# iagostorch/VVC-Affine-GPU

Measured on AMD Instinct MI355X. Metric: candidate CU-blocks/s at 1080p QP32; bit-exact CPMV/cost match vs reference, higher is better.
Workload: dtype int32; 1 GPU; 1920x1080 QP32, 2 frames, 2-CPMV affine only (FULL+HALF CUs); resolution=1920x1080, qp=32, sequence_frames=2, sequence_pairs=3, pocs_rank0=2, modes=2cp, parallelism=frame-shard x1 (a sequence of its own per rank)

## Files before the change

vvc-affine-gpu_amd/csrc/vame_engine.hip:

```cpp
#include <hip/hip_ext.h>
#include <hip/hip_runtime.h>

#include <algorithm>
#include <cstdio>
#include <cstdlib>
#include <cstring>
#include <vector>

#include "../../include/vame.h"
#include "vame_kernel.h"
#include "vame_bipred.h"
#include "vame_birefine.h"

#if VAME_SPLIT_TU
namespace vame {
VAME_2CP_KERNELS(extern)
}
#endif

using namespace vame;

static_assert(sizeof(vame_cpmvs) == 28, "Cpmvs layout (typedef.h)");
static_assert(sizeof(vame_cpmvs_dev) == 28, "Cpmvs layout (typedef.h)");
static_assert(sizeof(vame_mc_cu) == sizeof(McCu) && VAME_MC_MAX_CUS == kMcMaxCus, "vame_mc_cu layout");
static_assert(sizeof(vame_mc_bicu) == sizeof(McBiCu) && sizeof(McBiCu) == 80, "vame_mc_bicu layout");

static thread_local char g_hip_err[256] = "";

#define VAME_HIP(x)                                                               \
  do {                                                                            \
    hipError_t e_ = (x);                                                          \
    if (e_ != hipSuccess) {                                                       \
      snprintf(g_hip_err, sizeof(g_hip_err), "%s (%s:%d)", hipGetErrorString(e_), \
               __FILE__, __LINE__);                                               \
      return VAME_E_DEVICE;                                                       \
    }                                                                             \
  } while (0)

constexpr int kTimingClasses = 7;

struct vame_ctx {
  int device, W, H, nCtus, ctusPerRow;
  Item* dQuad = nullptr;
  int quadOff[4][3] = {}, quadN[4][3] = {};
  Item* dBig1 = nullptr;
  Item* dHalf = nullptr;
  Item* dHalfW = nullptr;
  Item* dHalfH = nullptr;
  int nBig1 = 0, nHalf = 0, nHalfW = 0, nHalfH = 0;
  int32_t* bestS = nullptr;
  size_t bestOff[4] = {0, 0, 0, 0};
  int maxPairs = kMaxPairs;
  hipEvent_t bestEv = nullptr;
  hipStream_t bestStream = nullptr;
  bool bestPending = false;
  int32_t* dOrder[2] = {nullptr, nullptr};
  int groupCombos[2] = {408, 408}, nChunks[2] = {1, 1}, cpp[2] = {0, 0};
  int streams = 2;
  hipStream_t side = nullptr;
  hipStream_t side2 = nullptr;
  hipEvent_t evFork = nullptr, evJoin = nullptr, evJoin2 = nullptr;
  int valueSync = 1;
  uint32_t* syncWord = nullptr;
  uint32_t joinSeq = 0;
  int timing = 0;
  bool prof = false;
  std::vector<std::pair<hipEvent_t, hipEvent_t>> ev[kTimingClasses];
  size_t evUsed[kTimingClasses] = {};
  std::vector<struct PackSeg> packSegs;
  struct PackSeg* dPackSegs = nullptr;
  size_t dPackCap = 0;
  hipEvent_t packEv = nullptr;
  int32_t* mcScratch = nullptr;
  int32_t* partScratch = nullptr;
  BiCand* biCands = nullptr;
  int32_t* biGroupCand = nullptr;
  int64_t* biPairSatd = nullptr;
// ... 76 lines not shown
    it.nCu = (int16_t)(t * stride + n);
  }
  return it;
}
Item make_coop_item(int rx, int ry, const std::vector<CuDesc>& cus, int threads) {
  return make_coop_item(rx, ry, std::vector<std::vector<CuDesc>>{cus}, threads);
}

Item make_auto_item(int rx, int ry, const std::vector<std::vector<CuDesc>>& tasks, int sbl) {
  Item it;
  memset(&it, 0, sizeof(it));
  it.rx = (int16_t)rx;
  it.ry = (int16_t)ry;
  it.coop = sbl == 2 ? 2 | 4 : 2;
  if (tasks.empty() || (int)tasks.size() > kMaxTasks) abort();
  it.nTasks = (int16_t)tasks.size();
  it.nCu = (int16_t)(tasks.size() * kTaskCu);
  for (size_t t = 0; t < tasks.size(); t++) {
    const int lanes = nsb_of(tasks[t][0]) / sbl;
    const int n = (int)tasks[t].size();
    for (auto& c : tasks[t])
      if (nsb_of(c) / sbl != lanes) abort();
    if (n * lanes > 64 || lanes < 16 || n > kTaskCu) abort();
    for (int i = 0; i < n; i++) set_slot(it.cu[t * kTaskCu + i], tasks[t][i]);
    it.cu[t * kTaskCu].taskCus = (uint8_t)n;
    it.cu[t * kTaskCu].taskLogL = (uint16_t)ilog2(lanes);
  }
  return it;
}

#ifndef VAME_Q2_TASKS
#define VAME_Q2_TASKS 16
#endif
size_t pack_autonomous(int qx, int qy, std::vector<CuDesc> cus, std::vector<Item>& out, int sbl) {
  const int perItem = sbl == 2 ? VAME_Q2_TASKS : kMaxTasks;
  std::stable_sort(cus.begin(), cus.end(),
                   [](const CuDesc& a, const CuDesc& b) { return nsb_of(a) > nsb_of(b); });
  std::vector<std::vector<CuDesc>> waves;
  for (auto& c : cus) {
    if (waves.empty() || nsb_of(waves.back()[0]) != nsb_of(c) || (int)waves.back().size() == kTaskCu ||
        (int)(waves.back().size() + 1) * nsb_of(c) / sbl > 64)
      waves.push_back({});
    waves.back().push_back(c);
  }
  for (size_t w = 0; w < waves.size(); w += perItem) {
    std::vector<std::vector<CuDesc>> grp(waves.begin() + w,
                                         waves.begin() + std::min(waves.size(), w + perItem));
    out.push_back(make_auto_item(qx, qy, grp, sbl));
  }
  return (waves.size() + perItem - 1) / perItem;
}

struct QuadSet {
  std::vector<Item> full, half, both;
};

void build_templates(std::vector<Item>& big, std::vector<Item>& halfItems, QuadSet& q1, QuadSet* q2) {
  for (int g = 0; g < kFullGroups; g++) {
    const int w = kFullW[g], h = kFullH[g], n = (kCtu * kCtu) / (w * h), cols = kCtu / w;
    if (w == 128 || h == 128) {
      std::vector<CuDesc> c;
      for (int k = 0; k < n; k++) c.push_back({(k % cols) * w, (k / cols) * h, w, h, 0, kFullStride[g] + k});
      if (w != h) {
        if (VAME_ABLATE & 256) continue;
        for (auto& cu : c) {
          Item it = make_coop_item(cu.x, cu.y, {cu}, Cfg<kKindHalf>::THREADS);
          it.rw = (int16_t)w;
          it.rh = (int16_t)h;
          halfItems.push_back(it);
        }
      } else {
        big.push_back(make_coop_item(0, 0, c, Cfg<kKindCtu>::THREADS));
      }
    }
  }
  const int max1 = q2 ? 16 : 64, min2 = 32, max2 = 128;
  struct Both {
    std::vector<Item> coop, autos;
    std::vector<int> rank;
  } both1, both2;
  for (int q = 0; q < 4; q++) {
    const int qx = (q & 1) * 64, qy = (q >> 1) * 64;
    auto inq = [&](int x, int y) { return x >= qx && x < qx + 64 && y >= qy && y < qy + 64; };
    std::vector<CuDesc> a1[2], a2[2];
    std::vector<std::vector<CuDesc>> coop[2];
    auto place = [&](const std::vector<CuDesc>& c, int align) {
      if (c.empty()) return;
      const int nsb = nsb_of(c[0]);
      if (nsb <= max1)
        a1[align].insert(a1[align].end(), c.begin(), c.end());
      else if (q2 && nsb >= min2 && nsb <= max2)
        a2[align].insert(a2[align].end(), c.begin(), c.end());
      else
        coop[align].push_back(c);
    };
    for (int g = 0; g < kFullGroups; g++) {
      const int w = kFullW[g], h = kFullH[g], n = (kCtu * kCtu) / (w * h), cols = kCtu / w;
      if (w == 128 || h == 128) continue;
      std::vector<CuDesc> c;
      for (int k = 0; k < n; k++) {
        const int x = (k % cols) * w, y = (k / cols) * h;
        if (inq(x, y)) c.push_back({x, y, w, h, 0, kFullStride[g] + k});
      }
      place(c, 0);
    }
    std::vector<CuDesc> halfBig;
    for (int g = 0; g < kHalfGroups; g++) {
      std::vector<CuDesc> c;
      for (int k = 0; k < kHalfN[g]; k++) {
        const int x = kHalfX8[g][k] * 8, y = kHalfY8[g][k] * 8;
        if (!inq(x, y)) continue;
        if (x + kHalfW[g] > qx + 64 || y + kHalfH[g] > qy + 64) abort();
        c.push_back({x, y, kHalfW[g], kHalfH[g], 1, kHalfStride[g] + k});
      }
      if (!c.empty() && nsb_of(c[0]) > max1 && !(q2 && nsb_of(c[0]) <= max2))
        halfBig.insert(halfBig.end(), c.begin(), c.end());
      else
        place(c, 1);
    }
    if (!halfBig.empty()) coop[1].push_back(halfBig);
    for (int al = 0; al < 2; al++) {
      std::vector<Item>& o1 = al ? q1.half : q1.full;
      if (!coop[al].empty()) o1.push_back(make_coop_item(qx, qy, coop[al], Cfg<kKindQuad>::THREADS));
      pack_autonomous(qx, qy, a1[al], o1, 1);
      if (q2) pack_autonomous(qx, qy, a2[al], al ? q2->half : q2->full, 2);
    }
    std::vector<std::vector<CuDesc>> t(coop[0]);
    t.insert(t.end(), coop[1].begin(), coop[1].end());
    if (!t.empty()) both1.coop.push_back(make_coop_item(qx, qy, t, Cfg<kKindQuad>::THREADS));
    for (int k = 0; k < (q2 ? 2 : 1); k++) {
      Both& b = k ? both2 : both1;
      std::vector<CuDesc> cus(k ? a2[0] : a1[0]);
      const std::vector<CuDesc>& h = k ? a2[1] : a1[1];
      cus.insert(cus.end(), h.begin(), h.end());
      const size_t n = pack_autonomous(qx, qy, cus, b.autos, k ? 2 : 1);
      for (size_t i = 0; i < n; i++) b.rank.push_back((int)i);
    }
  }
  for (int k = 0; k < (q2 ? 2 : 1); k++) {
    Both& b = k ? both2 : both1;
    std::vector<Item>& out = k ? q2->both : q1.both;
    out = b.coop;
    std::vector<size_t> idx(b.autos.size());
    for (size_t i = 0; i < idx.size(); i++) idx[i] = i;
    std::stable_sort(idx.begin(), idx.end(), [&](size_t x, size_t y) { return b.rank[x] < b.rank[y]; });
    for (size_t i : idx) out.push_back(b.autos[i]);
  }
}

size_t best_layout(const vame_ctx* c, int pairs, size_t off[4]) {
  const size_t per = (size_t)pairs * c->nCtus * 5;
  int nq2 = 0;
  for (int a = 0; a < 3; a++) nq2 = std::max({nq2, c->quadN[1][a], c->quadN[3][a]});
  off[0] = 0;
  off[1] = off[0] + per * c->nBig1 * Cfg<kKindCtu2>::NSB;
  off[2] = off[1] + per * c->nHalfW * Cfg<kKindHalf2W>::NSB;
  off[3] = off[2] + per * c->nHalfH * Cfg<kKindHalf2H>::NSB;
  return off[3] + per * nq2 * Cfg<kKindQuad2>::NSB;
}

int alloc_best(vame_ctx* c, int pairs) {
  if (c->bestS) {
    VAME_HIP(hipDeviceSynchronize());
    VAME_HIP(hipFree(c->bestS));
    c->bestS = nullptr;
  }
  c->bestPending = false;
  const size_t words = best_layout(c, pairs, c->bestOff);
  if (hipMalloc(&c->bestS, words * sizeof(int32_t)) != hipSuccess) {
    (void)hipGetLastError();
    c->bestS = nullptr;
    return VAME_E_NOMEM;
  }
  c->maxPairs = pairs;
  return VAME_OK;
}

void fill_common(KParams& kp, const vame_ctx* c, int extra) {
  kp.W = c->W;
  kp.H = c->H;
  kp.nCtus = c->nCtus;
// ... 180 lines not shown
      return VAME_OK;
    }
    if (half_merged(mode)) {
      KParams kh = kp;
      kh.items = c->dHalfW;
      kh.nItems = c->nHalfW + c->nHalfH;
      kh.bestS = c->bestS + c->bestOff[1];
      const unsigned grid = block_grid(c, 1, kh);
      hipEvent_t t0, t1;
      VAME_TRY(events(4, t0, t1));
      VAME_HIP(launch_kernel(kernel_for<kKindHalf2W + 100>(mode), grid, Cfg<kKindHalf2W>::THREADS, stream, t0,
                             t1, order_flag(), kh, capture));
      return VAME_OK;
    }
    for (int o = 0; o < 2; o++) {
      KParams kh = kp;
      kh.items = o ? c->dHalfH : c->dHalfW;
      kh.nItems = o ? c->nHalfH : c->nHalfW;
      kh.bestS = c->bestS + c->bestOff[1 + o];
      const unsigned grid = block_grid(c, 1, kh);
      hipEvent_t t0, t1;
      VAME_TRY(events(4 + o, t0, t1));
      VAME_HIP(launch_kernel(o ? kernel_for<kKindHalf2H>(mode) : kernel_for<kKindHalf2W>(mode), grid,
                             Cfg<kKindHalf2W>::THREADS, stream, t0, t1, order_flag(), kh, capture));
    }
    return VAME_OK;
  };
  const int aset = quadFull && quadHalf ? 2 : quadFull ? 0 : 1;
  auto quad = [&](const KParams& kp, int set, hipStream_t s) -> int {
    KParams kq = kp;
    kq.items = c->dQuad + c->quadOff[set][aset];
    kq.nItems = c->quadN[set][aset];
    kq.bestS = c->bestS + c->bestOff[3];
    const unsigned grid = block_grid(c, 0, kq);
    hipEvent_t t0, t1;
    VAME_TRY(events(set == 1 ? 6 : 0, t0, t1));
    if (set == 1)
      VAME_HIP(launch_kernel(kernel_for<kKindQuad2>(mode), grid, Cfg<kKindQuad2>::THREADS, s, t0, t1, order_flag(),
                             kq, capture));
    else
      VAME_HIP(launch_kernel(quad_kernel(c->prof, mode), grid, Cfg<kKindQuad>::THREADS, s, t0, t1, order_flag(),
                             kq, capture));
    return VAME_OK;
  };
  const bool anyQuad = quadFull || quadHalf;
  const bool kSplit = VAME_SPLIT == 1 || (VAME_SPLIT == 3 && mode != 1);
  auto quads = [&](const KParams& kp, hipStream_t s1) -> int {
    if (c->prof || VAME_SPLIT == 0) return quad(kp, 2, sQuad);
    if (!kSplit) return quad(kp, 3, sQuad);
    VAME_TRY(quad(kp, 1, sQuad));
    if (s1 == sQuad || !fork) VAME_TRY(quad(kp, 0, s1));
    return VAME_OK;
  };
  auto all = [&]() -> int {
    for (const KParams& kp : kps) {
      if (!fork && anyQuad) VAME_TRY(quads(kp, stream));
      if (bigItems) {
        VAME_TRY(big(kp));
        VAME_TRY(half(kp));
      }
      if (fork) {
        VAME_TRY(quads(kp, kQ1Side ? sQuad : stream));
        if (!kQ1Side && !c->prof && kSplit) VAME_TRY(quad(kp, 0, c->side2 ? c->side2 : stream));
      }
    }
    return fork ? join() : VAME_OK;
  };
// ... 42 lines not shown
    *ncu = (kCtu * kCtu) / (*w * *h);
    *stride = kFullStride[g];
    for (int k = 0; k < *ncu; k++) {
      xs[k] = (k % (kCtu / *w)) * *w;
      ys[k] = (k / (kCtu / *w)) * *h;
    }
    return VAME_OK;
  }
  if (align == 1 && g >= 0 && g < kHalfGroups) {
    *w = kHalfW[g];
    *h = kHalfH[g];
    *ncu = kHalfN[g];
    *stride = kHalfStride[g];
    for (int k = 0; k < *ncu; k++) {
      xs[k] = kHalfX8[g][k] * 8;
      ys[k] = kHalfY8[g][k] * 8;
    }
    return VAME_OK;
  }
  return VAME_E_INVALID;
}

int vame_create(vame_ctx** out, int device, int width, int height) {
  if (!out) return VAME_E_INVALID;
  *out = nullptr;
  const int nCtus = num_ctus(width, height);
  if (!nCtus) return VAME_E_INVALID;
  int ndev = 0;
  VAME_HIP(hipGetDeviceCount(&ndev));
  if (device < 0 || device >= ndev) return VAME_E_INVALID;
  DeviceGuard guard(device);
  VAME_HIP(guard.err);
  std::vector<Item> big1, hf, bigP, hfP;
  QuadSet qs[4];
  build_templates(big1, hf, qs[0], &qs[1]);
  build_templates(bigP, hfP, qs[2], nullptr);
  for (int a = 0; a < 3; a++) {
    const std::vector<Item>& v1 = a == 0 ? qs[0].full : a == 1 ? qs[0].half : qs[0].both;
    const std::vector<Item>& v2 = a == 0 ? qs[1].full : a == 1 ? qs[1].half : qs[1].both;
    std::vector<Item>& m = a == 0 ? qs[3].full : a == 1 ? qs[3].half : qs[3].both;
    for (const Item& it : v1)
      if (it.coop & 1) m.push_back(it);
    m.insert(m.end(), v2.begin(), v2.end());
    for (const Item& it : v1)
      if (!(it.coop & 1)) m.push_back(it);
  }
  std::vector<Item> hfw, hfh;
  for (const Item& it : hf) (it.cu[0].lw > it.cu[0].lh ? hfw : hfh).push_back(it);
  if (big1.size() != 1 || (!(VAME_ABLATE & 256) && (hfw.size() != 2 || hfh.size() != 2))) return VAME_E_INVALID;
  vame_ctx* c = new vame_ctx();
  c->device = device;
  c->W = width;
  c->H = height;
  c->nCtus = nCtus;
  c->ctusPerRow = (width + kCtu - 1) / kCtu;
  c->nBig1 = (int)big1.size();
  c->nHalf = (int)hf.size();
  c->nHalfW = (int)hfw.size();
  c->nHalfH = (int)hfh.size();
  std::vector<Item> quad;
  for (int k = 0; k < 4; k++)
    for (int a = 0; a < 3; a++) {
      const std::vector<Item>& v = a == 0 ? qs[k].full : a == 1 ? qs[k].half : qs[k].both;
      c->quadOff[k][a] = (int)quad.size();
      c->quadN[k][a] = (int)v.size();
      quad.insert(quad.end(), v.begin(), v.end());
    }
  c->streams = env_int("VAME_STREAMS", 2) == 1 ? 1 : 2;
  c->valueSync = env_int("VAME_SYNC", 1) != 0 ? 1 : 0;
  c->groupCombos[0] = c->groupCombos[1] = std::max(8, env_int("VAME_GROUP_COMBOS", 408));
  hipError_t e = hipSuccess;
  auto upload = [&](Item*& d, const std::vector<Item>& v) {
    if (e == hipSuccess && !v.empty()) e = hipMalloc(&d, v.size() * sizeof(Item));
    if (e == hipSuccess && !v.empty()) e = hipMemcpy(d, v.data(), v.size() * sizeof(Item), hipMemcpyHostToDevice);
  };
  upload(c->dQuad, quad);
  upload(c->dBig1, big1);
  upload(c->dHalf, hf);
  {
    std::vector<Item> hwh(hfw);
    hwh.insert(hwh.end(), hfh.begin(), hfh.end());
    upload(c->dHalfW, hwh);
    if (c->dHalfW) c->dHalfH = c->dHalfW + hfw.size();
  }
  for (int k = 0; k < 2 && e == hipSuccess; k++) {
    const std::vector<int32_t> order = build_order(nCtus, c->ctusPerRow, c->groupCombos[k], c->nChunks[k], c->cpp[k]);
    e = hipMalloc(&c->dOrder[k], order.size() * sizeof(int32_t));
    if (e == hipSuccess)
      e = hipMemcpy(c->dOrder[k], order.data(), order.size() * sizeof(int32_t), hipMemcpyHostToDevice);
  }
  if (e == hipSuccess && c->streams == 2) e = hipStreamCreateWithFlags(&c->side, hipStreamNonBlocking);
  if (e == hipSuccess && c->streams == 2 && VAME_SPLIT != 2 && VAME_Q1_SIDE == 2)
    e = hipStreamCreateWithFlags(&c->side2, hipStreamNonBlocking);
  if (e == hipSuccess) e = hipEventCreateWithFlags(&c->evJoin, hipEventDisableTiming);
  if (e == hipSuccess) e = hipEventCreateWithFlags(&c->evJoin2, hipEventDisableTiming);
  if (e == hipSuccess) e = hipEventCreateWithFlags(&c->evFork, hipEventDisableTiming);
  if (e == hipSuccess) e = hipEventCreateWithFlags(&c->bestEv, hipEventDisableTiming);
  if (e == hipSuccess && c->valueSync) {
    if (hipExtMallocWithFlags(reinterpret_cast<void**>(&c->syncWord), 8, hipMallocSignalMemory) != hipSuccess ||
        hipMemset(c->syncWord, 0, 8) != hipSuccess) {
      (void)hipGetLastError();
      if (c->syncWord) (void)hipFree(c->syncWord);
      c->syncWord = nullptr;
      c->valueSync = 0;
// ... 330 lines not shown
  if (reinterpret_cast<uintptr_t>(cur) & 7) return VAME_E_INVALID;
  BiRefineParams p;
  memset(&p, 0, sizeof(p));
  for (int r = 0; r < nrefs; r++) {
    if (!refs[r] || (reinterpret_cast<uintptr_t>(refs[r]) & 3)) return VAME_E_INVALID;
    p.refs[r] = refs[r];
  }
  if (c->prof) return VAME_E_UNSUPPORTED;
  if (max_cus == 0) return VAME_OK;
  DeviceGuard guard(c->device);
  VAME_HIP(guard.err);
  p.cur = cur;
  p.cus = reinterpret_cast<const McBiCu*>(cus);
  p.out = reinterpret_cast<McBiCu*>(out);
  p.cost = cost;
  p.bad = bad;
  p.maxCus = max_cus;
  p.nrefs = nrefs;
  p.W = c->W;
  p.H = c->H;
  p.rounds = rounds;
  p.lambda = lambda;
  p.ncusDev = ncus_dev;
  VAME_HIP(birefine_launch(p, (hipStream_t)stream));
  return VAME_OK;
}

int vame_template_coverage(int half128, int align, int32_t* hits, int32_t* items3) {
  if (!hits || (align != 0 && align != 1) || half128 == 0) return VAME_E_INVALID;
  std::vector<Item> big, hf, bigP, hfP;
  QuadSet q1, q2, qp;
  build_templates(big, hf, q1, &q2);
  build_templates(bigP, hfP, qp, nullptr);
  std::vector<Item> qf(q1.full), qh(q1.half), qb(q1.both);
  qf.insert(qf.end(), q2.full.begin(), q2.full.end());
  qh.insert(qh.end(), q2.half.begin(), q2.half.end());
  qb.insert(qb.end(), q2.both.begin(), q2.both.end());
  for (const std::vector<Item>* pv : {&qp.full, &qp.half, &qp.both}) {
    std::vector<int32_t> a((size_t)(align ? kHalfCusPerCtu : kFullCusPerCtu), 0),
        b((size_t)(align ? kHalfCusPerCtu : kFullCusPerCtu), 0);
    const std::vector<Item>& split = pv == &qp.full ? qf : pv == &qp.half ? qh : qb;
    for (int k = 0; k < 2; k++)
      for (const Item& it : k ? split : *pv)
        for (int i = 0; i < it.nCu; i++)
          if (it.cu[i].lw != 0 && it.cu[i].align == align) (k ? b : a)[it.cu[i].outOff]++;
    if (a != b) return VAME_E_INVALID;
  }
  const int n = align ? kHalfCusPerCtu : kFullCusPerCtu;
  std::vector<int32_t> both(n, 0);
  for (int i = 0; i < n; i++) hits[i] = 0;
  for (const auto* v : {&big, &hf, &qf, &qh, &qb})
    for (const Item& it : *v)
      for (int k = 0; k < it.nCu; k++) {
        const CuSlot& s = it.cu[k];
        if (s.lw == 0 || s.align != align) continue;
        if (s.outOff >= n) return VAME_E_INVALID;
        (v == &qb ? both[s.outOff] : hits[s.outOff])++;
      }
  for (const auto* v : {&big, &hf})
    for (const Item& it : *v)
      for (int k = 0; k < it.nCu; k++)
        if (it.cu[k].lw != 0 && it.cu[k].align == align) both[it.cu[k].outOff]++;
  for (int i = 0; i < n; i++)
    if (both[i] != hits[i]) return VAME_E_INVALID;
  if (items3) {
    items3[0] = (int32_t)qb.size();
// ... 157 lines not shown
    case VAME_E_DEVICE: return "HIP runtime error";
    case VAME_E_NOMEM: return "out of memory";
    case VAME_E_UNSUPPORTED: return "unsupported";
    default: return "unknown error";
  }
}

const char* vame_last_hip_error(void) { return g_hip_err; }

#if VAME_PHASE_TIMING
int vame_debug_phase_cycles(unsigned long long* out, int reset) {
  if (!out) return VAME_E_INVALID;
  VAME_HIP(hipDeviceSynchronize());
  VAME_HIP(hipMemcpyFromSymbol(out, HIP_SYMBOL(g_phase_cycles), sizeof(g_phase_cycles)));
  if (reset) {
    unsigned long long z[7 * kPhSlots] = {};
    VAME_HIP(hipMemcpyToSymbol(HIP_SYMBOL(g_phase_cycles), z, sizeof(z)));
  }
  return VAME_OK;
}
#endif
#if VAME_COUNT_PRED
int vame_debug_pred_count(unsigned long long* out20, int reset) {
  if (!out20) return VAME_E_INVALID;
  VAME_HIP(hipDeviceSynchronize());
  VAME_HIP(hipMemcpyFromSymbol(out20, HIP_SYMBOL(g_pred_count), sizeof(unsigned long long) * 20));
  if (reset) {
    unsigned long long z[20] = {};
    VAME_HIP(hipMemcpyToSymbol(HIP_SYMBOL(g_pred_count), z, sizeof(z)));
  }
  return VAME_OK;
}
#endif
const char* vame_version(void) { return "vame 0.1 (gfx950)"; }

}
```

vvc-affine-gpu_amd/csrc/vame_kernel.h:

```cpp
#pragma once
#include <hip/hip_runtime.h>

#include "vame_tables.h"

namespace vame {

constexpr int kMaxCu = 16;
constexpr int kMaxTasks = 16;
constexpr int kTaskCu = 4;
constexpr int kItemCu = kMaxTasks * kTaskCu;
constexpr int kThreads = 256;
constexpr int kNumMom = 24;
constexpr int kNumVal2 = 14;

struct vame_cpmvs_dev {
  int32_t ncps, ltx, lty, rtx, rty, lbx, lby;
};

struct CuSlot {
  uint8_t x, y;
  uint8_t lw : 4, lh : 4;
  uint8_t align : 1;
  uint8_t taskCus : 5;
  uint16_t outOff : 9;
// ... 86 lines not shown
#define PH_MARK(i) { const unsigned long long t_ = __builtin_amdgcn_s_memtime(); ph_acc[(i) + ph_off] += t_ - ph_t; ph_t = t_; }
__shared__ unsigned long long s_ph_blk[3];
__shared__ int s_ph_done;
#define PH_FLUSH { \
  if (lane == 0) { \
    for (int i_ = 0; i_ < 2 * kNumPhases; i_++) atomicAdd(&g_phase_cycles[KIND][i_], ph_acc[i_]); \
    const unsigned long long t1_ = __builtin_amdgcn_s_memtime(); \
    atomicMax(&s_ph_blk[1], t1_); \
    atomicAdd(&s_ph_blk[2], t1_ - ph_t0); \
    const int nw_ = (int)(blockDim.x >> 6); \
    if (atomicAdd(&s_ph_done, 1) == nw_ - 1) { \
      atomicAdd(&g_phase_cycles[KIND][2 * kNumPhases], (unsigned long long)nw_ * (s_ph_blk[1] - s_ph_blk[0])); \
      atomicAdd(&g_phase_cycles[KIND][2 * kNumPhases + 1], s_ph_blk[2]); \
      atomicAdd(&g_phase_cycles[KIND][2 * kNumPhases + 2], 1ull); \
      atomicAdd(&g_phase_cycles[KIND][2 * kNumPhases + 3], s_ph_blk[1] - s_ph_blk[0]); \
    } \
  } }
#define PH_INIT { if (tid == 0) { s_ph_blk[0] = ~0ull; s_ph_blk[1] = 0; s_ph_blk[2] = 0; s_ph_done = 0; } }
#define PH_START { if (lane == 0) atomicMin(&s_ph_blk[0], ph_t0); }
#elif defined(VAME_ISA_MARKS)
#define PH_DECL
#define PH_MARK(i) asm volatile("; PHASE_END " #i);
#define PH_FLUSH
#define PH_INIT
#define PH_START
#else
#define PH_DECL
#define PH_MARK(i)
#define PH_FLUSH
#define PH_INIT
#define PH_START
#endif

typedef short short2v __attribute__((ext_vector_type(2)));

__device__ __forceinline__ int clampi(int v, int lo, int hi) { return min(max(v, lo), hi); }
__device__ __forceinline__ int shl(int a, int s) { return (int)((unsigned)a << s); }
__device__ __forceinline__ short2v as_s2(unsigned v) { return __builtin_bit_cast(short2v, v); }
__device__ __forceinline__ unsigned as_u(short2v v) { return __builtin_bit_cast(unsigned, v); }
__device__ __forceinline__ int dot2(unsigned a, unsigned b, int acc) {
  return __builtin_amdgcn_sdot2(as_s2(a), as_s2(b), acc, false);
}
__device__ __forceinline__ unsigned pack16(int lo, int hi) {
  return __builtin_amdgcn_perm((unsigned)hi, (unsigned)lo, 0x05040100u);
}

__device__ __forceinline__ void wave_sync() {
  __builtin_amdgcn_fence(__ATOMIC_RELEASE, "wavefront");
  __builtin_amdgcn_wave_barrier();
  __builtin_amdgcn_fence(__ATOMIC_ACQUIRE, "wavefront");
}
__device__ __forceinline__ void phase_sync(bool coop) {
  if (coop)
    __syncthreads();
  else
    wave_sync();
}

__device__ __forceinline__ void clip_mv(int& x, int& y, int bx, int by, int W, int H) {
  x = clampi(x, shl(-128 - 8 - bx + 1, 4), shl(W + 8 - bx - 1, 4));
  y = clampi(y, shl(-128 - 8 - by + 1, 4), shl(H + 8 - by - 1, 4));
}

__device__ __forceinline__ bool spread_over_limit(int a, int b, int c, int d, bool six) {
  const int s4 = 4 << 11;
  int w = (abs(4 * a + s4) >> 11) + 9, h = (abs(4 * b) >> 11) + 9;
// ... 981 lines not shown
  using C = Cfg<KIND>;
  constexpr int REGION = C::REGION;
  (void)REGION;
  static_assert((C::TP * 2) % 16 == 0 && C::TILE_W % 8 == 0, "16-byte tile rows");
  constexpr int SBL = C::SBL;
  constexpr bool STASH = SBL == 2 && C::STASH;
  using Own = Lds<KIND, run2 && run3>;
  static_assert(sizeof(L::tile) >= sizeof(Own::tile) && sizeof(L::top) >= sizeof(Own::top) &&
                    sizeof(L::bestS) >= sizeof(Own::bestS) && sizeof(L::pred) >= sizeof(Own::pred) &&
                    sizeof(L::val) >= sizeof(Own::val) && sizeof(L::mat) >= sizeof(Own::mat) &&
                    sizeof(L::st) >= sizeof(Own::st) && sizeof(L::cu) >= sizeof(Own::cu),
                "LDS layout too small for this kernel class");
  uint16_t* s_tile = lds.tile;
  uint2* s_top = lds.top;
  uint2* s_bot = lds.bot;
  auto& s_bestS = lds.bestS;
  auto& s_pred = lds.pred;
  auto& s_val = lds.val;
  auto& s_mat = lds.mat;
  uint4* s_coef = lds.coef;
  uint8_t* s_eqmap = lds.eqmap;
  CuState* s_st = lds.st;
  CuSlot* s_cu = lds.cu;
  int* s_hdr = lds.hdr;
  __shared__ long long s_dup[(VAME_DUP & 4) ? kNumMom : 1];

  const int tid = threadIdx.x;
  [[maybe_unused]] const int lane = tid & 63;
  const int wv = tid >> 6;
  constexpr int ph_off = 0;
  (void)ph_off;
  PH_DECL
  PC_DECL

  const int b = blockIdx.x;
  const int gsz = p.nItems * p.groupPer;
  const int grp = b / gsz, gr = b % gsz;
  const int itemIdx = gr / p.groupPer;
  const int rest = gr % p.groupPer;
  const int pairIdx = (grp / p.nChunks) * p.groupPairs + rest / p.cpp;
  if (pairIdx >= p.nPairs) return;
  const int ctu = p.order[(grp % p.nChunks) * p.cpp + rest % p.cpp];
  if (ctu < 0) return;
  const PairArgs& pa = p.pair[pairIdx];
  const Item* it = p.items + itemIdx;
  const uint16_t* __restrict__ ref = pa.ref;
  const uint16_t* __restrict__ cur = pa.cur;
  const int W = p.W, H = p.H;
  const int ctuX = (ctu % p.ctusPerRow) * kCtu, ctuY = (ctu / p.ctusPerRow) * kCtu;

  const int tx0 = ctuX + (int)it->rx - C::MARGIN, ty0 = ctuY + (int)it->ry - C::MARGIN;
  const bool regionOut = tx0 + C::MARGIN >= W || ty0 + C::MARGIN >= H;
  const int tileW = KIND == kKindHalf ? (int)it->rw + 2 * C::MARGIN : C::TILE_W;
  const int tileH = KIND == kKindHalf ? (int)it->rh + 2 * C::MARGIN : C::TILE_H;
  const int CPR = tileW / 8;
  const int NCH = tileH * CPR;
  constexpr int PER = (C::TILE_H * (C::TILE_W / 8) + C::THREADS - 1) / C::THREADS;
  uint4 tv[PER];
  if constexpr ((VAME_DUP & 64) != 0) {
    if (!regionOut) {
#pragma unroll
      for (int j = 0; j < PER; j++) {
        const int ch = tid + j * C::THREADS;
        if (ch < NCH) {
          const int ty = ch / CPR, cx = clampi((ch % CPR) * 8 + tx0, 0, W - 8);
          tv[j] = *reinterpret_cast<const uint4*>(ref + (size_t)clampi(ty0 + ty, 0, H - 1) * W + cx);
// ... 18 lines not shown
#pragma unroll
          for (int m = 0; m < 8; m++) a[m] = row[clampi(fx + m, 0, W - 1)];
          tv[j] = make_uint4(a[0] | (a[1] << 16), a[2] | (a[3] << 16), a[4] | (a[5] << 16),
                             a[6] | (a[7] << 16));
        }
      }
    }
  }
  if (tid < C::ITEMCU) s_cu[tid] = it->cu[tid];
  if (tid < 48) s_coef[tid] = reinterpret_cast<const uint4*>(&kCoefTab)[tid];
  if (tid < 76) s_eqmap[tid] = kEqMap.v[tid];
  if (tid == 0) {
    s_hdr[0] = it->coop | (it->nTasks << 16);
    s_hdr[1] = 4;
  }
  for (int i = tid; i < C::MAXCU * kNumMom; i += C::THREADS) (&s_val[0][0])[i] = 0;
  PH_INIT
  if (!regionOut) {
#pragma unroll
    for (int j = 0; j < PER; j++) {
      const int ch = tid + j * C::THREADS;
      if (ch < NCH) *reinterpret_cast<uint4*>(&s_tile[(ch / CPR) * C::TP + (ch % CPR) * 8]) = tv[j];
    }
  }
  __syncthreads();
  PH_START
  const int hdr = __builtin_amdgcn_readfirstlane(s_hdr[0]);
  const int nTasks = (hdr >> 16) & 0xFF;
  const bool coop = C::COOP && (!C::AUTO || (hdr & 1) != 0);
  const bool claim = C::AUTO && (hdr & 2) != 0;
  PH_MARK(kPhStage)
  if (!coop && wv >= nTasks) {
    PH_FLUSH
    return;
  }

  const int tidItem = tid;
  for (int task = coop ? 0 : __builtin_amdgcn_readfirstlane(wv);;) {
    int tidTask = tidItem;
    opaque(tidTask);
    const int tid = tidTask, lane = tid & 63, wv = tid >> 6;
    const int lidx = coop ? tid : lane;
    const CuSlot t0 = s_cu[coop ? 0 : wv * kTaskCu];
    int cuB = coop ? 0 : wv * kTaskCu;
    int cuE = cuB + t0.taskCus;
    int logL = t0.taskLogL;
    cuB = __builtin_amdgcn_readfirstlane(cuB);
    cuE = __builtin_amdgcn_readfirstlane(cuE);
    logL = __builtin_amdgcn_readfirstlane(logL);
    const int logS = min(logL, 6);
    const int nCuW = coop ? (wv == 0 ? cuE : 0) : cuE - cuB;
    const int kLane = cuB + (lidx >> logL);
    const int myCu = kLane < cuE ? kLane : -1;
    Geo g;
    g.x = g.y = g.lw = g.lh = g.w = g.h = 0;
    const int local = lidx & ((1 << logL) - 1);
    int sbIdx = 0, sx = 0, sy = 0, sbCols = 1;
    bool active = false;
    if (myCu >= 0) {
      const CuSlot cs = s_cu[myCu];
      g.lw = cs.lw;
      g.lh = cs.lh;
      g.w = 1 << g.lw;
      g.h = 1 << g.lh;
      g.x = ctuX + cs.x;
      g.y = ctuY + cs.y;
// ... 449 lines not shown
    using I2 = std::integral_constant<int, 2>;
    using I3 = std::integral_constant<int, 3>;
    using T = std::true_type;
    using F = std::false_type;
    using KeepS = std::integral_constant<bool, run3>;
    if (C::COOP && coop) {
      if constexpr (C::COOP) {
        if constexpr (run2) run_pass(I2{}, T{}, KeepS{});
        if constexpr (run3) run_pass(I3{}, T{}, F{});
      }
    } else {
      if constexpr (run2) run_pass(I2{}, F{}, KeepS{});
      if constexpr (run3) run_pass(I3{}, F{}, F{});
    }
    if (!C::QUAD) break;
    int next = task + (coop ? 1 : 4);
    if (claim) {
      int v = 0;
      if (lane == 0) v = atomicAdd(&s_hdr[1], 1);
      next = __builtin_amdgcn_readfirstlane(v);
    }
    if (next >= nTasks) break;
    if (coop) {
      if (tid < kTaskCu) s_cu[tid] = s_cu[min(next, C::ITEMCU / kTaskCu - 1) * kTaskCu + tid];
      __syncthreads();
    } else {
      if (lane < kTaskCu) s_cu[wv * kTaskCu + lane] = s_cu[min(next, C::ITEMCU / kTaskCu - 1) * kTaskCu + lane];
      wave_sync();
    }
    task = next;
  }
  PH_FLUSH
  PC_FLUSH
}

__device__ __forceinline__ bool quad_item_sbl2(const KParams& p) {
  const int b = blockIdx.x;
  const int gr = b % (p.nItems * p.groupPer);
  return (p.items[gr / p.groupPer].coop & 4) != 0;
}
#ifndef VAME_SPLIT
#define VAME_SPLIT 3
#endif
template <int MODE>
constexpr bool kQuadMerged = VAME_SPLIT == 2 || (VAME_SPLIT == 3 && MODE == 1);
template <int MODE>
__global__ __launch_bounds__(kThreads) __attribute__((amdgpu_waves_per_eu(4))) void affine_me_quad(
    KParams p) {
  __shared__ Lds<kKindQuad, MODE == 3> lds;
  if constexpr (kQuadMerged<MODE>) {
    if (quad_item_sbl2(p)) {
      affine_me_body<kKindQuad2, false, MODE>(p, lds);
      return;
    }
  }
  affine_me_body<kKindQuad, false, MODE>(p, lds);
}
template <int MODE>
__global__ __launch_bounds__(kThreads) __attribute__((amdgpu_waves_per_eu(4))) void affine_me_quad2(
    KParams p) {
  __shared__ Lds<kKindQuad2, MODE == 3> lds;
  affine_me_body<kKindQuad2, false, MODE>(p, lds);
}
template <int MODE>
__global__ __launch_bounds__(512) __attribute__((amdgpu_waves_per_eu(4))) void affine_me_ctu2(KParams p) {
  __shared__ Lds<kKindCtu2, MODE == 3> lds;
// ... 6 lines not shown
}
template <int MODE>
__global__ __launch_bounds__(256) __attribute__((amdgpu_waves_per_eu(4))) void affine_me_half2h(KParams p) {
  __shared__ Lds<kKindHalf2H, MODE == 3> lds;
  affine_me_body<kKindHalf2H, false, MODE>(p, lds);
}
template <int MODE>
__global__ __launch_bounds__(256) __attribute__((amdgpu_waves_per_eu(4))) void affine_me_half2(KParams p) {
  __shared__ Lds<kKindHalf2H, MODE == 3> lds;
  const int gr = blockIdx.x % (p.nItems * p.groupPer);
  const Item& it = p.items[gr / p.groupPer];
  if (it.rw > it.rh)
    affine_me_body<kKindHalf2W, false, MODE>(p, lds);
  else
    affine_me_body<kKindHalf2H, false, MODE>(p, lds);
}
template <int MODE>
__global__ __launch_bounds__(kThreads) __attribute__((amdgpu_waves_per_eu(4))) void affine_me_quad_prof(
    KParams p) {
  __shared__ Lds<kKindQuad, MODE == 3> lds;
  affine_me_body<kKindQuad, true, MODE>(p, lds);
}
template <int MODE>
__global__ __launch_bounds__(1024) void affine_me_ctu_prof(KParams p) {
  __shared__ Lds<kKindCtu, MODE == 3> lds;
  affine_me_body<kKindCtu, true, MODE>(p, lds);
}
template <int MODE>
__global__ __launch_bounds__(512) __attribute__((amdgpu_waves_per_eu(4))) void affine_me_half_prof(KParams p) {
  __shared__ Lds<kKindHalf, MODE == 3> lds;
  affine_me_body<kKindHalf, true, MODE>(p, lds);
}

#if VAME_COUNT_PRED || VAME_PHASE_TIMING
#define VAME_SPLIT_TU 0
#else
#define VAME_SPLIT_TU 1
#endif
#define VAME_2CP_KERNELS(X)                 \
  X template __global__ void affine_me_quad<1>(KParams);   \
  X template __global__ void affine_me_quad2<1>(KParams);  \
  X template __global__ void affine_me_ctu2<1>(KParams);   \
  X template __global__ void affine_me_half2<1>(KParams);  \
  X template __global__ void affine_me_half2w<1>(KParams); \
  X template __global__ void affine_me_half2h<1>(KParams);

struct McCu {
  int32_t x, y, w, h, ref;
  int32_t ncps, ltx, lty, rtx, rty, lbx, lby;
};
constexpr int kMcMaxCus = 1 << 20;
constexpr size_t kMcScratchWords = (size_t)kMcMaxCus + 1 + 1024;
struct McParams {
  const uint16_t* cur;
  const uint16_t* refs[4];
  const McCu* cus;
  uint16_t* pred;
  int64_t* cost;
  int32_t* bad;
  int32_t* offs;
  int32_t* blockSum;
  int ncus, nrefs, W, H;
  float lambda;
  const int32_t* ncusDev;
};
hipError_t mc_launch(const McParams& p, bool prof, hipStream_t stream);

// ... 23 lines not shown
```

Measured before the change: 231.0 million CU-blocks/s.

## Split last autonomous quadrant items into smaller tail items to cut wave-tail idle

Adds a graded packing of autonomous quadrant work items where the final item of each group is cut into smaller pieces, and builds separate full/half item sets for it. At launch, the graded item set is chosen when the grid is small relative to resident quad-kernel capacity (or when forced via env). The goal is less idle slot time at the end of the quadrant kernel, when few long workgroups remain. It also adds workgroup timeline tracing and A/B profiling scripts. The cost is more items and per-item staging overhead.

```diff
diff --git a/profiles/tail_ab.py b/profiles/tail_ab.py
--- /dev/null
+++ b/profiles/tail_ab.py
@@ -0,0 +1,88 @@
+#!/usr/bin/env python3
+import argparse
+import os
+import sys
+
+REPO = os.path.dirname(os.path.dirname(os.path.abspath(__file__)))
+sys.path.insert(0, os.path.join(REPO, "vvc-affine-gpu_amd"))
+
+import numpy as np
+import torch
+
+
+def timed(fn, calls, warmup):
+    for _ in range(warmup):
+        fn()
+    torch.cuda.synchronize()
+    t0, t1 = torch.cuda.Event(enable_timing=True), torch.cuda.Event(enable_timing=True)
+    t0.record()
+    for _ in range(calls):
+        fn()
+    t1.record()
+    torch.cuda.synchronize()
+    return t0.elapsed_time(t1) / calls * 1e3
+
+
+def main():
+    ap = argparse.ArgumentParser(description=__doc__, formatter_class=argparse.RawDescriptionHelpFormatter)
+    ap.add_argument("--reps", type=int, default=3)
+    args = ap.parse_args()
+    from vame import synth
+    from vame._lib import LIB_PATH
+    from vame.engine import Engine
+    from vame.hostlogic import lambda_for_poc
+
+    W, H, qp = 1920, 1080, 32
+    dev = torch.device("cuda", 0)
+    orig, recon = synth.synth_sequence(W, H, 10, qp)
+    up = lambda f: torch.from_numpy(f.view(np.int16)).to(dev)
+    o, r = [up(f) for f in orig], [up(f) for f in recon]
+    settings = {"plain": "0", "graded": "1", "rule": None}
+    eng = {}
+    for name, v in settings.items():
+        if v is None:
+            os.environ.pop("VAME_TAIL_SPLIT", None)
+        else:
+            os.environ["VAME_TAIL_SPLIT"] = v
+        eng[name] = Engine(W, H, 0)
+    os.environ.pop("VAME_TAIL_SPLIT", None)
+
+    def batch_case(e, pairs, modes=1):
+        jobs, left = [], pairs
+        for k in range(10):
+            n = min(4, k + 1, left)
+            if n == 0:
+                break
+            jobs.append((o[k], [r[k - i] for i in range(n)], lambda_for_poc(qp, k + 1), e.alloc_poc(n, modes)))
+            left -= n
+        assert left == 0
+        return lambda: e.affine_me_batch(jobs, modes, 0)
+
+    def poc_case(e):
+        res = e.alloc_poc(4, 3)
+        refs = [r[3 - i] for i in range(4)]
+        lam = lambda_for_poc(qp, 4)
+        return lambda: e.affine_me_poc(o[4], refs, lam, modes=3, out=res)
+
+    cases = [(f"2-CP batch, {p:2d} pairs", lambda e, p=p: batch_case(e, p), max(20, 300 // p)) for p in (3, 8, 16, 32)]
+    cases.append(("2+3-CP poc call, 4 refs", poc_case, 100))
+    cases += [(f"2+3-CP batch, {p:2d} pairs", lambda e, p=p: batch_case(e, p, 3), max(10, 240 // p)) for p in (8, 16, 32)]
+    print(f"# {torch.cuda.get_device_name(0)}; {os.path.basename(LIB_PATH)}; us per call, "
+          f"{args.reps} interleaved repetitions")
+    for title, make, calls in cases:
+        fns = {name: make(e) for name, e in eng.items()}
+        t = {name: [] for name in fns}
+        for _ in range(args.reps):
+            for name, fn in fns.items():
+                t[name].append(timed(fn, calls, 10))
+        base = float(np.mean(t["plain"]))
+        for name in fns:
+            print(f"{title} | {name:6s} | " + " ".join(f"{x:9.1f}" for x in t[name]) +
+                  f" | mean {np.mean(t[name]):9.1f} | vs plain {100 * (np.mean(t[name]) / base - 1):+.2f} %")
+        sys.stdout.flush()
+    for e in eng.values():
+        e.close()
+
+
+if __name__ == "__main__":
+    main()
diff --git a/profiles/wg_timeline.py b/profiles/wg_timeline.py
--- /dev/null
+++ b/profiles/wg_timeline.py
@@ -0,0 +1,143 @@
+#!/usr/bin/env python3
+import argparse
+import ctypes
+import os
+import sys
+
+REPO = os.path.dirname(os.path.dirname(os.path.abspath(__file__)))
+os.environ.setdefault("VAME_LIB", os.path.join(REPO, "vvc-affine-gpu_amd", "lib", "libvame_wgtrace.so"))
+sys.path.insert(0, os.path.join(REPO, "vvc-affine-gpu_amd"))
+
+import numpy as np
+import torch
+
+CAP = 1 << 18
+TICK_US = 0.01
+KERNEL = {1: {0: "affine_me_quad", 6: "affine_me_quad", 3: "affine_me_ctu2", 4: "affine_me_half2",
+              5: "affine_me_half2"},
+          3: {0: "affine_me_quad", 6: "affine_me_quad2", 3: "affine_me_ctu2", 4: "affine_me_half2w",
+              5: "affine_me_half2h"}}
+
+
+def read_trace(L):
+    buf = (ctypes.c_ulonglong * (3 * CAP))()
+    n = L.vame_debug_wg_trace(buf, CAP, 1)
+    if n < 0:
+        raise RuntimeError(f"vame_debug_wg_trace: {n}")
+    if n == CAP:
+        raise RuntimeError("the trace table is full")
+    w = np.frombuffer(buf, dtype=np.uint64, count=3 * n).reshape(n, 3)
+    key, inv = np.unique(w[:, 0], return_inverse=True)
+    t0 = np.full(len(key), np.iinfo(np.uint64).max, np.uint64)
+    t1 = np.zeros(len(key), np.uint64)
+    np.minimum.at(t0, inv, w[:, 1])
+    np.maximum.at(t1, inv, w[:, 2])
+    return np.stack([key & np.uint64(0xFFFFFFFF), t0, t1], 1)
+
+
+def describe(name, rec, mode, out):
+    kind = (rec[:, 0] & 0xFF).astype(int)
+    item = ((rec[:, 0] >> 8) & 0xFFFF).astype(int)
+    flags = ((rec[:, 0] >> 24) & 7).astype(int)
+    t0 = rec[:, 1].astype(np.int64)
+    t1 = rec[:, 2].astype(np.int64)
+    base = t0.min()
+    a, b = (t0 - base) * TICK_US, (t1 - base) * TICK_US
+    out.append(f"== {name}: {len(rec)} workgroups, {b.max():.1f} us from the first entry to the last exit")
+    kern = np.array([KERNEL[mode][k] for k in kind])
+    ends = {}
+    for kn in sorted(set(kern), key=lambda k: a[kern == k].min()):
+        m = kern == kn
+        ka, kb, ki, kf = a[m], b[m], item[m], flags[m]
+        ends[kn] = kb.max()
+        ev = np.concatenate([np.stack([ka, np.ones_like(ka)], 1), np.stack([kb, -np.ones_like(kb)], 1)])
+        ev = ev[np.lexsort((ev[:, 1], ev[:, 0]))]
+        res = np.cumsum(ev[:, 1])
+        slots = int(res.max())
+        out.append(f"-- {kn}: {m.sum()} workgroups, first entry {ka.min():.1f} us, last entry (end of dispatch) "
+                   f"{ka.max():.1f} us, last exit {kb.max():.1f} us, at most {slots} resident")
+        out.append("   resident workgroups against time (us: count), every 25 us and at the end of dispatch:")
+        ts = sorted(set(np.arange(0, kb.max() + 25, 25).tolist() + [float(ka.max())]))
+        line = []
+        for t in ts:
+            i = np.searchsorted(ev[:, 0], t, side="right") - 1
+            line.append(f"{t:.0f}:{int(res[i]) if i >= 0 else 0}")
+        for i in range(0, len(line), 12):
+            out.append("     " + "  ".join(line[i:i + 12]))
+        out.append("   duration per item index (us): item [body] n  min / median / p90 / max   entries from .. to")
+        for it in sorted(set(ki)):
+            s = ki == it
+            d = kb[s] - ka[s]
+            body = "coop" if kf[s][0] & 1 else "SBL2" if kf[s][0] & 4 else "SBL1"
+            out.append(f"     {it:3d} [{body}] {s.sum():5d}  {d.min():6.1f} / {np.median(d):6.1f} / "
+                       f"{np.percentile(d, 90):6.1f} / {d.max():6.1f}   {ka[s].min():7.1f} .. {ka[s].max():7.1f}")
+        tl, te = ka.max(), kb.max()
+        busy = np.clip(np.minimum(kb, te) - np.maximum(ka, tl), 0, None).sum()
+        last = np.argsort(ka)[-min(1024, len(ka)):]
+        dl = (kb - ka)[last]
+        out.append(f"   after the last dispatch: {te - tl:.1f} us to the kernel's end, {slots * (te - tl) - busy:.0f} "
+                   f"slot-us idle of {slots * (te - tl):.0f} ({slots} slots); the last {len(last)} workgroups "
+                   f"dispatched ran {np.median(dl):.1f} us (median), {dl.min():.1f} .. {dl.max():.1f}")
+    last_k = max(ends, key=ends.get)
+    out.append(f"-- the launch ends with {last_k} (" + ", ".join(f"{k} {v:.1f}" for k, v in ends.items()) + " us)")
+    qd = a[kern == "affine_me_quad"].max()
+    for kn in ends:
+        if kn.startswith("affine_me_half2"):
+            m = kern == kn
+            out.append(f"   {kn} at the end of affine_me_quad's dispatch ({qd:.1f} us): "
+                       f"{int((a[m] > qd).sum())} workgroups not yet started, {int((b[m] > qd).sum())} not yet finished")
+    out.append("")
+
+
+def main():
+    ap = argparse.ArgumentParser(description=__doc__, formatter_class=argparse.RawDescriptionHelpFormatter)
+    ap.add_argument("--out", required=True)
+    args = ap.parse_args()
+    from vame import synth
+    from vame._lib import lib
+    from vame.engine import Engine
+    from vame.hostlogic import lambda_for_poc
+
+    L = lib()
+    if not hasattr(L, "vame_debug_wg_trace"):
+        sys.exit("the library is not a VAME_WG_TRACE build (make variant NAME=wgtrace DEFS=-DVAME_WG_TRACE=1)")
+    W, H, qp = 1920, 1080, 32
+    dev = torch.device("cuda", 0)
+    orig, recon = synth.synth_sequence(W, H, 5, qp)
+    up = lambda f: torch.from_numpy(f.view(np.int16)).to(dev)
+    o, r = [up(f) for f in orig], [up(f) for f in recon]
+    out = [f"# {torch.cuda.get_device_name(0)}; VAME_TAIL_SPLIT={os.environ.get('VAME_TAIL_SPLIT', '(unset)')}; "
+           f"{os.path.basename(os.environ['VAME_LIB'])}", ""]
+
+    eng = Engine(W, H, 0)
+    jobs = [(o[0], [r[0]], lambda_for_poc(qp, 1), eng.alloc_poc(1, 1)),
+            (o[1], [r[1], r[0]], lambda_for_poc(qp, 2), eng.alloc_poc(2, 1))]
+    for _ in range(5):
+        eng.affine_me_batch(jobs, 1, 0)
+    torch.cuda.synchronize()
+    read_trace(L)
+    eng.affine_me_batch(jobs, 1, 0)
+    torch.cuda.synchronize()
+    describe("c2 step (3 pairs, 2-CP only)", read_trace(L), 1, out)
+    eng.close()
+
+    eng = Engine(W, H, 0)
+    eng.set_max_pairs(4)
+    refs = [r[3 - k] for k in range(4)]
+    res = eng.alloc_poc(4, 3)
+    for _ in range(3):
+        eng.affine_me_poc(o[4], refs, lambda_for_poc(qp, 4), modes=3, out=res)
+    torch.cuda.synchronize()
+    read_trace(L)
+    eng.affine_me_poc(o[4], refs, lambda_for_poc(qp, 4), modes=3, out=res)
+    torch.cuda.synchronize()
+    describe("affine_me_poc, 4 references, 2+3 CP", read_trace(L), 3, out)
+    eng.close()
+
+    with open(args.out, "w") as f:
+        f.write("\n".join(out))
+    print("\n".join(out))
+
+
+if __name__ == "__main__":
+    main()
diff --git a/vvc-affine-gpu_amd/csrc/vame_engine.hip b/vvc-affine-gpu_amd/csrc/vame_engine.hip
--- a/vvc-affine-gpu_amd/csrc/vame_engine.hip
+++ b/vvc-affine-gpu_amd/csrc/vame_engine.hip
@@ -42,7 +42,8 @@
 struct vame_ctx {
   int device, W, H, nCtus, ctusPerRow;
   Item* dQuad = nullptr;
-  int quadOff[4][3] = {}, quadN[4][3] = {};
+  int quadOff[6][3] = {}, quadN[6][3] = {};
+  int tailSplit = -1, residentQuad = 0;
   Item* dBig1 = nullptr;
   Item* dHalf = nullptr;
   Item* dHalfW = nullptr;
@@ -185,7 +186,7 @@
 #ifndef VAME_Q2_TASKS
 #define VAME_Q2_TASKS 16
 #endif
-size_t pack_autonomous(int qx, int qy, std::vector<CuDesc> cus, std::vector<Item>& out, int sbl) {
+size_t pack_autonomous(int qx, int qy, std::vector<CuDesc> cus, std::vector<Item>& out, int sbl, int cut = 0) {
   const int perItem = sbl == 2 ? VAME_Q2_TASKS : kMaxTasks;
   std::stable_sort(cus.begin(), cus.end(),
                    [](const CuDesc& a, const CuDesc& b) { return nsb_of(a) > nsb_of(b); });
@@ -196,19 +197,29 @@
       waves.push_back({});
     waves.back().push_back(c);
   }
+  size_t n = 0;
   for (size_t w = 0; w < waves.size(); w += perItem) {
-    std::vector<std::vector<CuDesc>> grp(waves.begin() + w,
-                                         waves.begin() + std::min(waves.size(), w + perItem));
-    out.push_back(make_auto_item(qx, qy, grp, sbl));
-  }
-  return (waves.size() + perItem - 1) / perItem;
+    const size_t e = std::min(waves.size(), w + perItem);
+    const bool last = e == waves.size();
+    const size_t first = last && cut < 0 && e - w > (size_t)-cut ? e - w - (size_t)-cut : 0;
+    const size_t step = last && cut > 0 ? (size_t)cut : (size_t)perItem;
+    for (size_t v = w; v < e; n++) {
+      const size_t ve = std::min(e, v + (v == w && first ? first : step));
+      std::vector<std::vector<CuDesc>> grp(waves.begin() + v, waves.begin() + ve);
+      out.push_back(make_auto_item(qx, qy, grp, sbl));
+      v = ve;
+    }
+  }
+  return n;
 }
 
 struct QuadSet {
   std::vector<Item> full, half, both;
 };
 
-void build_templates(std::vector<Item>& big, std::vector<Item>& halfItems, QuadSet& q1, QuadSet* q2) {
+void build_templates(std::vector<Item>& big, std::vector<Item>& halfItems, QuadSet& q1, QuadSet* q2,
+                     int grade = 0) {
+  const int cut1 = grade == 3 ? -4 : grade >= 1 ? 4 : 0, cut2 = grade == 2 ? 8 : 0;
   for (int g = 0; g < kFullGroups; g++) {
     const int w = kFullW[g], h = kFullH[g], n = (kCtu * kCtu) / (w * h), cols = kCtu / w;
     if (w == 128 || h == 128) {
@@ -231,7 +242,7 @@
   struct Both {
     std::vector<Item> coop, autos;
     std::vector<int> rank;
-  } both1, both2;
+  } both1, both2, one1[2], one2[2];
   for (int q = 0; q < 4; q++) {
     const int qx = (q & 1) * 64, qy = (q >> 1) * 64;
     auto inq = [&](int x, int y) { return x >= qx && x < qx + 64 && y >= qy && y < qy + 64; };
@@ -273,6 +284,16 @@
     }
     if (!halfBig.empty()) coop[1].push_back(halfBig);
     for (int al = 0; al < 2; al++) {
+      if (grade) {
+        if (!coop[al].empty())
+          one1[al].coop.push_back(make_coop_item(qx, qy, coop[al], Cfg<kKindQuad>::THREADS));
+        for (int k = 0; k < (q2 ? 2 : 1); k++) {
+          Both& b = k ? one2[al] : one1[al];
+          const size_t n = pack_autonomous(qx, qy, k ? a2[al] : a1[al], b.autos, k ? 2 : 1, k ? cut2 : cut1);
+          for (size_t i = 0; i < n; i++) b.rank.push_back((int)i);
+        }
+        continue;
+      }
       std::vector<Item>& o1 = al ? q1.half : q1.full;
       if (!coop[al].empty()) o1.push_back(make_coop_item(qx, qy, coop[al], Cfg<kKindQuad>::THREADS));
       pack_autonomous(qx, qy, a1[al], o1, 1);
@@ -286,20 +307,47 @@
       std::vector<CuDesc> cus(k ? a2[0] : a1[0]);
       const std::vector<CuDesc>& h = k ? a2[1] : a1[1];
       cus.insert(cus.end(), h.begin(), h.end());
-      const size_t n = pack_autonomous(qx, qy, cus, b.autos, k ? 2 : 1);
+      const size_t n = pack_autonomous(qx, qy, cus, b.autos, k ? 2 : 1, k ? cut2 : cut1);
       for (size_t i = 0; i < n; i++) b.rank.push_back((int)i);
     }
   }
-  for (int k = 0; k < (q2 ? 2 : 1); k++) {
-    Both& b = k ? both2 : both1;
-    std::vector<Item>& out = k ? q2->both : q1.both;
+  auto emit = [](const Both& b, std::vector<Item>& out) {
     out = b.coop;
     std::vector<size_t> idx(b.autos.size());
     for (size_t i = 0; i < idx.size(); i++) idx[i] = i;
     std::stable_sort(idx.begin(), idx.end(), [&](size_t x, size_t y) { return b.rank[x] < b.rank[y]; });
     for (size_t i : idx) out.push_back(b.autos[i]);
-  }
-}
+  };
+  for (int k = 0; k < (q2 ? 2 : 1); k++) {
+    emit(k ? both2 : both1, k ? q2->both : q1.both);
+    if (grade) {
+      emit(k ? one2[0] : one1[0], k ? q2->full : q1.full);
+      emit(k ? one2[1] : one1[1], k ? q2->half : q1.half);
+    }
+  }
+}
+
+QuadSet merged_set(const QuadSet& q1, const QuadSet& q2) {
+  QuadSet m;
+  for (int a = 0; a < 3; a++) {
+    const std::vector<Item>& v1 = a == 0 ? q1.full : a == 1 ? q1.half : q1.both;
+    const std::vector<Item>& v2 = a == 0 ? q2.full : a == 1 ? q2.half : q2.both;
+    std::vector<Item>& o = a == 0 ? m.full : a == 1 ? m.half : m.both;
+    for (const Item& it : v1)
+      if (it.coop & 1) o.push_back(it);
+    o.insert(o.end(), v2.begin(), v2.end());
+    for (const Item& it : v1)
+      if (!(it.coop & 1)) o.push_back(it);
+  }
+  return m;
+}
+
+#ifndef VAME_TAIL_GRADE
+#define VAME_TAIL_GRADE 1
+#endif
+#ifndef VAME_TAIL_ROUNDS
+#define VAME_TAIL_ROUNDS 20
+#endif
 
 size_t best_layout(const vame_ctx* c, int pairs, size_t off[4]) {
   const size_t per = (size_t)pairs * c->nCtus * 5;
@@ -546,7 +594,18 @@
     kq.items = c->dQuad + c->quadOff[set][aset];
     kq.nItems = c->quadN[set][aset];
     kq.bestS = c->bestS + c->bestOff[3];
-    const unsigned grid = block_grid(c, 0, kq);
+    unsigned grid = block_grid(c, 0, kq);
+    if (((set == 3 && mode == 1 && c->tailSplit > 0) || set == 0) && c->tailSplit != 0 &&
+        (c->tailSplit > 0 || grid <= (unsigned)VAME_TAIL_ROUNDS * (unsigned)c->residentQuad)) {
+      const int gset = set == 3 ? 4 : 5;
+      kq.items = c->dQuad + c->quadOff[gset][aset];
+      kq.nItems = c->quadN[gset][aset];
+      grid = block_grid(c, 0, kq);
+    }
+#if VAME_WG_TRACE
+    fprintf(stderr, "vame: quadrant launch mode %d set %d: %d items, %d pairs, grid %u (%.1f rounds of %d)\n", mode,
+            set, kq.nItems, kq.nPairs, grid, (double)grid / c->residentQuad, c->residentQuad);
+#endif
     hipEvent_t t0, t1;
     VAME_TRY(events(set == 1 ? 6 : 0, t0, t1));
     if (set == 1)
@@ -655,18 +714,15 @@
   DeviceGuard guard(device);
   VAME_HIP(guard.err);
   std::vector<Item> big1, hf, bigP, hfP;
-  QuadSet qs[4];
+  QuadSet qs[6];
   build_templates(big1, hf, qs[0], &qs[1]);
   build_templates(bigP, hfP, qs[2], nullptr);
-  for (int a = 0; a < 3; a++) {
-    const std::vector<Item>& v1 = a == 0 ? qs[0].full : a == 1 ? qs[0].half : qs[0].both;
-    const std::vector<Item>& v2 = a == 0 ? qs[1].full : a == 1 ? qs[1].half : qs[1].both;
-    std::vector<Item>& m = a == 0 ? qs[3].full : a == 1 ? qs[3].half : qs[3].both;
-    for (const Item& it : v1)
-      if (it.coop & 1) m.push_back(it);
-    m.insert(m.end(), v2.begin(), v2.end());
-    for (const Item& it : v1)
-      if (!(it.coop & 1)) m.push_back(it);
+  qs[3] = merged_set(qs[0], qs[1]);
+  {
+    std::vector<Item> bigG, hfG;
+    QuadSet g2;
+    build_templates(bigG, hfG, qs[5], &g2, VAME_TAIL_GRADE);
+    qs[4] = merged_set(qs[5], g2);
   }
   std::vector<Item> hfw, hfh;
   for (const Item& it : hf) (it.cu[0].lw > it.cu[0].lh ? hfw : hfh).push_back(it);
@@ -682,7 +738,7 @@
   c->nHalfW = (int)hfw.size();
   c->nHalfH = (int)hfh.size();
   std::vector<Item> quad;
-  for (int k = 0; k < 4; k++)
+  for (int k = 0; k < 6; k++)
     for (int a = 0; a < 3; a++) {
       const std::vector<Item>& v = a == 0 ? qs[k].full : a == 1 ? qs[k].half : qs[k].both;
       c->quadOff[k][a] = (int)quad.size();
@@ -692,7 +748,15 @@
   c->streams = env_int("VAME_STREAMS", 2) == 1 ? 1 : 2;
   c->valueSync = env_int("VAME_SYNC", 1) != 0 ? 1 : 0;
   c->groupCombos[0] = c->groupCombos[1] = std::max(8, env_int("VAME_GROUP_COMBOS", 408));
+  c->tailSplit = env_int("VAME_TAIL_SPLIT", -1);
+  c->tailSplit = c->tailSplit < 0 ? -1 : c->tailSplit != 0;
   hipError_t e = hipSuccess;
+  {
+    int perCu = 0, cus = 0;
+    e = hipOccupancyMaxActiveBlocksPerMultiprocessor(&perCu, quad_kernel(false, 1), Cfg<kKindQuad>::THREADS, 0);
+    if (e == hipSuccess) e = hipDeviceGetAttribute(&cus, hipDeviceAttributeMultiprocessorCount, device);
+    c->residentQuad = std::max(1, perCu * cus);
+  }
   auto upload = [&](Item*& d, const std::vector<Item>& v) {
     if (e == hipSuccess && !v.empty()) e = hipMalloc(&d, v.size() * sizeof(Item));
     if (e == hipSuccess && !v.empty()) e = hipMemcpy(d, v.data(), v.size() * sizeof(Item), hipMemcpyHostToDevice);
@@ -1089,6 +1153,46 @@
   QuadSet q1, q2, qp;
   build_templates(big, hf, q1, &q2);
   build_templates(bigP, hfP, qp, nullptr);
+  if (half128 == 2) {
+    std::vector<Item> bigG, hfG;
+    QuadSet g1, g2;
+    build_templates(bigG, hfG, g1, &g2, VAME_TAIL_GRADE);
+    const QuadSet m = merged_set(q1, q2), gm = merged_set(g1, g2);
+    const int n = align ? kHalfCusPerCtu : kFullCusPerCtu;
+    auto cover = [&](const std::vector<Item>& v, std::vector<int32_t>& h) {
+      for (const Item& it : v) {
+        if (it.nTasks < 1 || it.nTasks > kMaxTasks) return false;
+        for (int k = 0; k < it.nCu; k++) {
+          const CuSlot& s = it.cu[k];
+          if (s.lw == 0 || s.align != align) continue;
+          if (s.outOff >= n) return false;
+          h[s.outOff]++;
+        }
+      }
+      return true;
+    };
+    std::vector<int32_t> onealign(n, 0);
+    for (int a = 0; a < 3; a++) {
+      const std::vector<Item>* plain[2] = {a == 0 ? &m.full : a == 1 ? &m.half : &m.both,
+                                           a == 0 ? &q1.full : a == 1 ? &q1.half : &q1.both};
+      const std::vector<Item>* graded[2] = {a == 0 ? &gm.full : a == 1 ? &gm.half : &gm.both,
+                                            a == 0 ? &g1.full : a == 1 ? &g1.half : &g1.both};
+      for (int k = 0; k < 2; k++) {
+        std::vector<int32_t> hp(n, 0), hg(n, 0);
+        if (!cover(*plain[k], hp) || !cover(*graded[k], hg) || hp != hg) return VAME_E_INVALID;
+        if (k == 0 && a == align) onealign = hg;
+        if (graded[k]->empty() || graded[k]->back().nTasks > 4) return VAME_E_INVALID;
+      }
+    }
+    if (!cover(big, onealign) || !cover(hf, onealign)) return VAME_E_INVALID;
+    for (int i = 0; i < n; i++) hits[i] = onealign[i];
+    if (items3) {
+      items3[0] = (int32_t)gm.both.size();
+      items3[1] = (int32_t)big.size();
+      items3[2] = (int32_t)hf.size();
+    }
+    return VAME_OK;
+  }
   std::vector<Item> qf(q1.full), qh(q1.half), qb(q1.both);
   qf.insert(qf.end(), q2.full.begin(), q2.full.end());
   qh.insert(qh.end(), q2.half.begin(), q2.half.end());
@@ -1312,6 +1416,21 @@
   return VAME_OK;
 }
 #endif
+#if VAME_WG_TRACE
+int vame_debug_wg_trace(unsigned long long* out, int cap, int reset) {
+  if (!out || cap < 0) return VAME_E_INVALID;
+  VAME_HIP(hipDeviceSynchronize());
+  unsigned n = 0;
+  VAME_HIP(hipMemcpyFromSymbol(&n, HIP_SYMBOL(g_wg_trace_n), sizeof(n)));
+  n = std::min({n, kWgTraceCap, (unsigned)cap});
+  if (n) VAME_HIP(hipMemcpyFromSymbol(out, HIP_SYMBOL(g_wg_trace), (size_t)n * 3 * sizeof(unsigned long long)));
+  if (reset) {
+    const unsigned z = 0;
+    VAME_HIP(hipMemcpyToSymbol(HIP_SYMBOL(g_wg_trace_n), &z, sizeof(z)));
+  }
+  return (int)n;
+}
+#endif
 const char* vame_version(void) { return "vame 0.1 (gfx950)"; }
 
 }
diff --git a/vvc-affine-gpu_amd/csrc/vame_kernel.h b/vvc-affine-gpu_amd/csrc/vame_kernel.h
--- a/vvc-affine-gpu_amd/csrc/vame_kernel.h
+++ b/vvc-affine-gpu_amd/csrc/vame_kernel.h
@@ -142,6 +142,29 @@
 #define PH_START
 #endif
 
+#ifndef VAME_WG_TRACE
+#define VAME_WG_TRACE 0
+#endif
+#if VAME_WG_TRACE
+constexpr unsigned kWgTraceCap = 1u << 18;
+__device__ unsigned long long g_wg_trace[kWgTraceCap][3];
+__device__ unsigned int g_wg_trace_n;
+#define WT_DECL const unsigned long long wt_t0 = wall_clock64();
+#define WT_FLUSH { \
+  if (lane == 0) { \
+    const unsigned slot_ = atomicAdd(&g_wg_trace_n, 1u); \
+    if (slot_ < kWgTraceCap) { \
+      g_wg_trace[slot_][0] = (unsigned long long)(KIND | (itemIdx << 8) | ((hdr & 7) << 24)) | \
+                             ((unsigned long long)blockIdx.x << 32); \
+      g_wg_trace[slot_][1] = wt_t0; \
+      g_wg_trace[slot_][2] = wall_clock64(); \
+    } \
+  } }
+#else
+#define WT_DECL
+#define WT_FLUSH
+#endif
+
 typedef short short2v __attribute__((ext_vector_type(2)));
 
 __device__ __forceinline__ int clampi(int v, int lo, int hi) { return min(max(v, lo), hi); }
@@ -1189,6 +1212,7 @@
   (void)ph_off;
   PH_DECL
   PC_DECL
+  WT_DECL
 
   const int b = blockIdx.x;
   const int gsz = p.nItems * p.groupPer;
@@ -1273,6 +1297,7 @@
   PH_MARK(kPhStage)
   if (!coop && wv >= nTasks) {
     PH_FLUSH
+    WT_FLUSH
     return;
   }
 
@@ -1788,6 +1813,7 @@
   }
   PH_FLUSH
   PC_FLUSH
+  WT_FLUSH
 }
 
 __device__ __forceinline__ bool quad_item_sbl2(const KParams& p) {
@@ -1860,7 +1886,7 @@
   affine_me_body<kKindHalf, true, MODE>(p, lds);
 }
 
-#if VAME_COUNT_PRED || VAME_PHASE_TIMING
+#if VAME_COUNT_PRED || VAME_PHASE_TIMING || VAME_WG_TRACE
 #define VAME_SPLIT_TU 0
 #else
 #define VAME_SPLIT_TU 1
```

After: 231.1 million CU-blocks/s (median of 4 runs). About the same (+0.0%).
